# tsbertalan/openmg

Measured on AMD Instinct MI355X. Metric: V-cycles/sec, 3-D 7-point Poisson 256^3, higher is better.
Workload: dtype f64

## Files before the change

### openmg_amd/csrc/common.h

```cpp
#pragma once
#include <hip/hip_runtime.h>

#include <algorithm>
#include <array>
#include <cstdint>
#include <cstdio>
#include <cstdlib>
#include <cstring>
#include <new>
#include <stdexcept>
#include <memory>
#include <string>
#include <type_traits>
#include <utility>
#include <vector>

#include "../../include/openmg_hip.h"

#if !defined(OMG_EXPERIMENTS) && (defined(PLANE_STORE_AUX) || defined(PLANE_LA_BIG) || defined(PLANE_LA) || defined(PLANE_WAVE_SYNC) || \
                                  defined(PLANE_WSYNC_F32) || defined(S27_COEF_AUX) || defined(S27_SG) || defined(S27_WAVES) ||        \
                                  defined(MARCH_NAP_MAX) || defined(OMG_ROWBLK_NNZ) || defined(PLANE_SETPRIO))
#error "tuning switches are experiments: add -DOMG_EXPERIMENTS"
#endif

// ... 476 lines not shown
    DevBuf<int32_t> gi_ptr, gi_idx;
    DevBuf<V> gi_val;
    DevBuf<int32_t> ig_ptr, ig_idx;
    DevBuf<V> ig_val;
    DevBuf<V> y, xg;
    int sx = 0, sy = 0, sz = 0;
    DevBuf<double> sine, lambda;
    size_t bytes = 0;
    bool retain_workspace = false;
    DevBuf<double> ws_aug, ws_inv64, ws_keep;
    int64_t bs = 0;
    int K = 0;
    DevBuf<V> dinv;
    DevBuf<int32_t> lo_ptr, lo_idx, up_ptr, up_idx;
    DevBuf<V> lo_val, up_val;
    DevBuf<V> z;
    void build_chain(const HostCsr &A, const int32_t *d_ptr, const int32_t *d_idx, const double *d_val, hipStream_t s);
    void build(const HostCsr &A, hipStream_t s);
    bool build_sine(const HostCsr &A, hipStream_t s);
    void solve(const V *b, V *x, hipStream_t s) const;
    bool cube16() const;
};

constexpr int PROJECT_MAX_WG = 2048;
constexpr int PROJECT_SCRATCH = PROJECT_MAX_WG + 1;
template <typename V>
void launch_project_mean(V *x, int64_t n, double *scratch, hipStream_t s);

constexpr int MARCH_FACE_PAD = 72;
struct MarchGeom {
    int nx = 0, ny = 0, nz = 0;
    int TJ = 0, TK = 0;
    int ntj = 0, ntk = 0, n_tiles = 0;
    int T = 0, n_grp = 0;
    int n_pat = 0;
};
template <typename V>
struct MarchPlan {
    MarchGeom g;
    DevBuf<uint32_t> codes;
    DevBuf<V> coef;
    DevBuf<uint32_t> sync;
    DevBuf<int32_t> order;
    DevBuf<V> faceJ, faceK;
    bool line1 = false;
    DevBuf<V> tri;
    bool per_row = false;
    DevBuf<V> rowc;
    bool line_scan = false;
    int scan_c = 0, scan_g = 0;
    DevBuf<uint8_t> rowcode;
    DevBuf<V> face_scan;
    bool build(const omg_csr &A, hipStream_t s);
    void sweep(V *x, const V *b, hipStream_t s) const;
    bool timed_out(hipStream_t s) const;
};

struct DevCsrPlain {
    int64_t n_rows = 0, n_cols = 0, nnz = 0;
    DevBuf<int32_t> indptr, indices;
    DevBuf<double> data;
};
void galerkin_chain_device(const omg_csr &A0, int dim, const int64_t *shape, int n_restrictions, std::vector<DevCsrPlain> &A,
                           std::vector<DevCsrPlain> &R, hipStream_t s);
void galerkin_chain_semi_device(const omg_csr &A0, int dim, const int64_t *shape, int n_restrictions, const int *factors, int64_t min_size,
                                std::vector<DevCsrPlain> &A, std::vector<DevCsrPlain> &R, std::vector<int> &used, hipStream_t s);
void semicoarsen_rule(int dim, const int64_t *shape, const double *sums, const int64_t *counts, int line_axis, int level, int *factors);
void check_factors(int dim, const int64_t *ext, const int *f, int level);
HostCsr download_csr(const DevCsrPlain &M, hipStream_t s);
bool rap_aggregation_device(const DevCsrPlain &R, const DevCsrPlain &A, DevCsrPlain &C, hipStream_t s);

bool is_plain_aggregation(const omg_csr &R, int64_t nx, int64_t ny, int64_t nz, double &w);

constexpr int PLANE_EDGE = 4;
struct PlaneGeom {
    int nx = 0, ny = 0, nz = 0;
    int hx = 0;
    int z_base = 0, z_end = 0, kv0 = 0, kv1 = 0, kc_off = 0, nzc = 0;
    int TX = 0, TY = 0, LZ = 0;
    int PX = 0, PY = 0;
    int ntx = 0, nty = 0, ntz = 0, n_wg = 0;
    int threads = 0;
    size_t lds_bytes = 0;
    double c[7] = {0, 0, 0, 0, 0, 0, 0};
    double w = 0.0;
    double over = 1.0;
    bool dim2 = false;
    bool jacobi = false;
    double omega = 1.0;
    bool block = false;
    bool la2 = true;
};
template <typename V>
struct PlanePlan {
    PlaneGeom g;
    DevBuf<double> partials;
    uint32_t *status = nullptr;
    bool build(const omg_csr &A, const omg_csr &R, Ordering &ord, bool jacobi = false, double omega = 1.0);
    bool build_device(const DevCsrPlain &A, int nx, int ny, int nz, double w, Ordering &ord, bool jacobi, double omega, hipStream_t s);
    bool finish_geometry(int64_t nx, int64_t ny, int64_t nz, const double (&c)[7], double w, bool jacobi, double omega);
    void spmv(const V *x, V *y, hipStream_t s) const;
    HostCsr operator_csr() const;
    HostCsr restriction_csr() const;
    void build_slab(int nx, int ny, int nz_own, int ghost, int ghost_c, bool first, bool last, const double (&c)[7], double w);
    struct Peer {
        V *x[2] = {nullptr, nullptr};
        V *bc[2] = {nullptr, nullptr};
        int64_t shift = 0, cshift = 0;
        int planes = 0, cplanes = 0;
        int zc_lo = 0, zc_hi = 0;
        const uint32_t *wait_flag[4] = {nullptr, nullptr, nullptr, nullptr};
        uint32_t wait_seq[4] = {0, 0, 0, 0};
        bool fused_wait = true;
        uint32_t *done = nullptr;
        uint32_t *flag[2] = {nullptr, nullptr};
        uint32_t seq = 0;
        uint32_t *status = nullptr;
        uint32_t spin = 1u << 21;
    };
    struct Coarse {
        const int32_t *map = nullptr;
        V *b = nullptr;
        V *x = nullptr;
        const V *diag = nullptr;
        int first_end = 0;
        const V *e = nullptr;
    };
    void tune(V *x, V *tmp, const V *b, const Coarse &c, hipStream_t s, bool finest = true);
    float time_pair(V *x, V *tmp, const V *b, const Coarse &c, hipStream_t s, bool finest, int pairs);
    enum { PART_ALL = 0, PART_EDGE = 1, PART_INNER = 2 };
    bool can_split() const {
        return !g.dim2 && !g.block && !(g.la2 && g.threads <= 128) && (g.z_end - g.z_base) >= 3 * PLANE_EDGE;
    }
    int split_partials() const {
        const int nzo = g.z_end - g.z_base;
        return nzo >= 3 * PLANE_EDGE ? g.ntx * g.nty * (2 + (nzo - 2 * PLANE_EDGE + g.LZ - 1) / g.LZ) : g.n_wg;
    }
    struct Gate {
        const uint32_t *flag[4] = {nullptr, nullptr, nullptr, nullptr};
        uint32_t seq[4] = {0, 0, 0, 0};
        uint32_t *status = nullptr;
        uint32_t spin = 1u << 21;
    };
    bool can_gate() const { return can_split() && 2 * g.ntx * g.nty <= 192 && (g.z_end - g.z_base) >= 96; }
    int gate_lz() const;
    int gate_partials() const;
    void down(const V *x_old, V *x_new, const V *b, bool x_zero, const Coarse &c, hipStream_t s, const Peer *peer = nullptr,
              bool sweep = true, int part = PART_ALL, const Gate *gate = nullptr) const;
    void up(const V *x_old, V *x_new, const V *b, const Coarse &c, double *out, hipStream_t s, const Peer *peer = nullptr,
            bool sweep = true, int part = PART_ALL, const Gate *gate = nullptr) const;
};

template <typename V>
struct TailUp {
    const PlaneGeom *top = nullptr, *mid = nullptr;
    const V *x_old = nullptr, *b = nullptr, *mid_x_old = nullptr, *mid_b = nullptr;
    V *x_new = nullptr, *mid_x_new = nullptr;
    const int32_t *cmap = nullptr;
    const V *cb = nullptr;
    V *cx = nullptr;
    const double *tables = nullptr, *lambda = nullptr;
    bool sweep = true;
};
bool tail_up_level(const PlaneGeom &g, int nxc, int nyc, int nzc);
template <typename V>
void launch_tail_up(const TailUp<V> &u, hipStream_t s);
// ... 123 lines not shown
```

### openmg_amd/csrc/plane.hip

```cpp
#include <algorithm>
#include <array>
#include <atomic>
#include <cmath>
#include <cstring>
#include <map>
#include <mutex>
#include <thread>
#include <type_traits>

#include "common.h"
#include "peer_wait.h"
#include "sine_cube16.h"

#if defined(OMG_PLANE_STAMPS) || defined(OMG_PLANE_DBGARGS)
#define OMG_PLANE_DBG_ON 1
#endif

namespace omg {
namespace {

#ifndef PLANE_STORE_AUX
#define PLANE_STORE_AUX 2
#endif
typedef unsigned v2u __attribute__((ext_vector_type(2)));
// ... 166 lines not shown
__device__ __forceinline__ void quotients(const V (&n)[4], V c, V r, bool fast, V (&q)[4]) {
    if (sizeof(V) == 8 && fast) {
        bool bad = false;
#pragma unroll
        for (int i = 0; i < 4; ++i) {
            const V q0 = n[i] * r;
            q[i] = madd(madd(-c, q0, n[i]), r, q0);
            bad = bad || !plain_numerator(n[i]);
        }
        if (__builtin_amdgcn_ballot_w64(bad) == 0) return;
    }
#pragma unroll
    for (int i = 0; i < 4; ++i) q[i] = n[i] / c;
}

template <typename V>
struct Inline {
    V imx, ipx, imy, ipy;
};
template <typename V>
__device__ __forceinline__ Inline<V> in_line(int rule, const P2<V> &O, V nb) {
    Inline<V> r;
    r.imx = rule ? O.x : nb;
    r.ipx = rule ? O.y : O.x;
    r.imy = rule ? O.y : O.x;
    r.ipy = rule ? nb : O.y;
    return r;
}

__device__ __forceinline__ void peer_done(uint32_t *done, uint32_t n_wg, uint32_t *const (&flag)[2], uint32_t seq) {
    __builtin_amdgcn_fence(__ATOMIC_RELEASE, "workgroup");
    __syncthreads();
    if (threadIdx.x == 0) {
        const uint32_t before = __hip_atomic_fetch_add(done, 1u, __ATOMIC_RELAXED, __HIP_MEMORY_SCOPE_AGENT);
        if (before == n_wg - 1) {
            __hip_atomic_store(done, 0u, __ATOMIC_RELAXED, __HIP_MEMORY_SCOPE_AGENT);
            for (int i = 0; i < 2; ++i)
                if (flag[i]) __hip_atomic_store(flag[i], seq, __ATOMIC_RELAXED, __HIP_MEMORY_SCOPE_SYSTEM);
        }
    }
}
__global__ void plane_wait_kernel(const uint32_t *f0, const uint32_t *f1, const uint32_t *f2, const uint32_t *f3,
                                  uint32_t s0, uint32_t s1, uint32_t s2, uint32_t s3, uint32_t *status, uint32_t spin) {
    if (threadIdx.x == 0) {
        peer_wait(f0, s0, status, spin);
        peer_wait(f1, s1, status, spin);
        peer_wait(f2, s2, status, spin);
        peer_wait(f3, s3, status, spin);
    }
}

template <typename V, int MODE, bool NORM, bool XZ, int LA, bool PEER = false, int MAXT = 512, bool FIRST = false, bool SWEEP = true, bool MIRROR = false>
__global__ __launch_bounds__(MAXT) void plane_kernel(const PlaneKArgs<V> a) {
    static_assert(!MIRROR || (MODE == 1 && !PEER && !FIRST && !XZ), "mirrored march: up passes of whole grids");
#ifdef OMG_PLANE_STAMPS
    const unsigned long long st_entry = __builtin_amdgcn_s_memtime();
#endif
    extern __shared__ __attribute__((aligned(16))) unsigned char plane_smem[];
    V *const lds = reinterpret_cast<V *>(plane_smem);
    __shared__ double s_red[8];
    __shared__ int s_step[8];
    if (threadIdx.x < 8) s_step[threadIdx.x] = 0;

    const int PX = a.PX, PY = a.PY;
    const int S = 2 * PX + 4;
    const int BUF = (2 * PY + 2) * S;
    const int t = int(threadIdx.x);
    const bool live = t < PX * PY;
    const int px = live ? t % PX : 0, py = live ? t / PX : 0;
    int L = int(blockIdx.x);
    int nwg = int(gridDim.x);
    const bool edge_wg = !PEER && a.edge_wg0 > 0 && L >= a.edge_wg0;
    if (!PEER && a.edge_wg0 > 0) {
        if (edge_wg) { L -= a.edge_wg0; nwg = 1; }
        else nwg = a.edge_wg0;
    }
    if ((nwg & 7) == 0) L = (L & 7) * (nwg >> 3) + (L >> 3);
    const int nxy = a.ntx * a.nty;
    const int tz = L / nxy, rem = L - tz * nxy;
    const int ty = rem / a.ntx, tx = rem - ty * a.ntx;
    const int z0 = edge_wg ? (tz ? a.z_end - PLANE_EDGE : a.z_base) : a.zc_base + tz * a.zc_stride;
    const int z1 = edge_wg ? z0 + PLANE_EDGE : min(a.zc_end, z0 + a.zc_len);
    const int q = tx * a.TXq + px - 1;
    const int ja = ty * a.TY + 2 * py - 4;
    const bool vx0 = live && q >= 0 && 2 * q < a.hx, vx1 = live && q >= 0 && 2 * q + 1 < a.hx;
    const bool vl[2] = {ja >= 0 && ja < a.ny, ja + 1 >= 0 && ja + 1 < a.ny};
    const bool inner = live && px >= 1 && px <= PX - 2 && py >= 2 && py <= PY - 3;
    const int ps = a.ny * a.hx;
    const int lb[2] = {ja * a.hx + 2 * q, (ja + 1) * a.hx + 2 * q};

    const __amdgpu_buffer_rsrc_t xs = __builtin_amdgcn_make_buffer_rsrc(const_cast<V *>(a.x_old), 0, a.vec_bytes, 0x00020000);
    const __amdgpu_buffer_rsrc_t bs = __builtin_amdgcn_make_buffer_rsrc(const_cast<V *>(a.b), 0, a.vec_bytes, 0x00020000);
    const __amdgpu_buffer_rsrc_t ws = __builtin_amdgcn_make_buffer_rsrc(a.x_new, 0, a.vec_bytes, 0x00020000);
    const __amdgpu_buffer_rsrc_t es = __builtin_amdgcn_make_buffer_rsrc(const_cast<V *>(MODE == 1 ? a.ec : a.cdiag), 0, a.cvec_bytes, 0x00020000);
    const __amdgpu_buffer_rsrc_t ms = __builtin_amdgcn_make_buffer_rsrc(const_cast<int32_t *>(a.cmap), 0, a.cmap_bytes, 0x00020000);

    constexpr int W = int(sizeof(V));
    const bool vcell = vl[0] && vx0;
    V c1a = ja > 0 ? a.c1 : V(0);
    V c5b = ja + 2 < a.ny ? a.c5 : V(0);
    V c2x = q > 0 ? a.c2 : V(0);
    V c4x = 2 * q + 1 < a.hx ? a.c4 : V(0);
    V c4y = 2 * q + 2 < a.hx ? a.c4 : V(0);
    unsigned lbo[2] = {vcell ? unsigned(lb[0] * W) : unsigned(OOB), vcell ? unsigned(lb[1] * W) : unsigned(OOB)};
    unsigned lso[2] = {(vcell && inner) ? unsigned(lb[0] * W) : unsigned(OOB), (vcell && inner) ? unsigned(lb[1] * W) : unsigned(OOB)};
    asm volatile("" : "+v"(c1a), "+v"(c5b), "+v"(c2x), "+v"(c4x), "+v"(c4y));
    asm volatile("" : "+v"(lbo[0]), "+v"(lbo[1]), "+v"(lso[0]), "+v"(lso[1]));
    const bool oddx = (a.hx & 1) != 0;

    auto head = [&](int l, int v, int rule, V km, V jm, V im) -> V {
        V sum = madd(a.c0, km, V(0));
        sum = madd(l == 0 ? c1a : a.c1, jm, sum);
        return madd((v == 0 && rule == 0) ? c2x : a.c2, im, sum);
    };
    auto tail = [&](int l, int v, int rule, V sum, V d, V ip, V jp, V kp) -> V {
        sum = madd(a.c3, d, sum);
        sum = madd(rule == 0 ? a.c4 : (v == 0 ? c4x : c4y), ip, sum);
        sum = madd(l == 1 ? c5b : a.c5, jp, sum);
        return madd(a.c6, kp, sum);
    };

    auto zphys = [&](int k) -> int { return MIRROR ? a.nz - 1 - k : k; };
    auto cplane = [&](int kc) -> int { return MIRROR ? (a.nz / 2 - 1 + a.kc_off) - kc : kc + a.kc_off; };
    auto plane_off = [&](int colour, int k) -> unsigned {
        return (k >= a.kv0 && k < a.kv1) ? unsigned(((colour ? a.nr : 0) + zphys(k) * ps) * W) : unsigned(OOB);
    };
    auto fetch = [&](const __amdgpu_buffer_rsrc_t &rs, int colour, int k, int l) -> P2<V> {
        unsigned po = plane_off(colour, k);
        asm volatile("" : "+s"(po));
        return bload2(rs, int(lbo[l] + po), V(0));
    };
    auto fetch_at = [&](const __amdgpu_buffer_rsrc_t &rs, unsigned po, int l) -> P2<V> { return bload2(rs, int(lbo[l] + po), V(0)); };
    auto fetch_x = [&](int colour, int k, int l) -> P2<V> {
        if (XZ) return {V(0), V(0)};
        return fetch(xs, colour, k, l);
    };
    constexpr int XAUX = sizeof(V) == 8 ? PLANE_STORE_AUX : 0;
    auto put_pair = [&](const __amdgpu_buffer_rsrc_t &rs, unsigned off, const P2<V> &v) {
#ifdef OMG_PLANE_DBG_ON
        if (a.dbg & 1) return;
#endif
        if (oddx) {
            bstore1<XAUX>(rs, int(off), v.x);
            bstore1<XAUX>(rs, int(vx1 ? off + unsigned(W) : unsigned(OOB)), v.y);
        } else {
            bstore2(rs, int(off), v, true);
        }
    };
    const bool vcoarse = vcell && (MODE == 1 || inner);
    const int cbase = (ja >> 1) * a.nxc + 2 * q;
    unsigned cb4 = vcoarse ? unsigned(cbase * 4) : unsigned(OOB);
    unsigned lmx = vcoarse ? 0u : unsigned(OOB), lmy = (vcoarse && vx1) ? 0u : unsigned(OOB);
    asm volatile("" : "+v"(cb4), "+v"(lmx), "+v"(lmy));
    const v2u none = {unsigned(OOB), unsigned(OOB)};
    auto slots_request = [&](int kc, bool want) -> v2u {
        kc = cplane(kc);
        const bool ok = want && a.cmap && kc >= 0 && kc < a.nzc;
        return __builtin_amdgcn_raw_buffer_load_b64(ms, int(cb4 + (ok ? unsigned(kc * a.nyc * a.nxc * 4) : unsigned(OOB))), 0, 0);
    };
    auto slots_commit = [&](const v2u &m, int kc, bool want) -> v2u {
        kc = cplane(kc);
        const bool ok = want && kc >= 0 && kc < a.nzc;
        const unsigned u = ok ? 0u : unsigned(OOB), cn = ok ? unsigned(kc * a.nyc * a.nxc * W) : 0u;
        const unsigned s0_ = a.cmap ? m.x * unsigned(W) : cn + cb4 * unsigned(W / 4), s1_ = a.cmap ? m.y * unsigned(W) : cn + cb4 * unsigned(W / 4) + unsigned(W);
        return v2u{s0_ | lmx | u, s1_ | lmy | u};
    };
    auto coarse_slots = [&](int kc) -> v2u { return slots_commit(slots_request(kc, true), kc, true); };
    auto coarse_vals = [&](const v2u &sl) -> P2<V> { return {bload1(es, int(sl.x), V(0)), bload1(es, int(sl.y), V(0))}; };
    auto prolonged = [&](const P2<V> &x, const P2<V> &e) -> P2<V> {
        return {x.x + madd(a.wp, e.x, V(0)), x.y + madd(a.wp, e.y, V(0))};
    };

    const V rc3 = refined_rcp(a.c3);
    const bool fast = a.fast_div != 0;
    const int row_a = 1 + 2 * py, col = 2 + 2 * px;
    const int idx[2] = {row_a * S + col, (row_a + 1) * S + col};
    for (int i = t; i < 6 * BUF; i += int(blockDim.x)) lds[i] = V(0);
    if (((PEER && a.fused_wait) || edge_wg) && t == 0) {
#pragma unroll
        for (int i = 0; i < 4; ++i) peer_wait(a.wait_flag[i], a.wait_seq[i], a.status, a.spin);
    }
    __syncthreads();
    int pside = 0;
    if (PEER) {
        const bool lo = z0 < a.z_base + 2 * PEER_CPLANES, hi = z1 > a.z_end - 2 * PEER_CPLANES;
        pside = (lo && a.peer_x[0] ? 1 : 0) | (hi && a.peer_x[1] ? 2 : 0) | (lo && a.peer_bc[0] ? 4 : 0) | (hi && a.peer_bc[1] ? 8 : 0);
    }
    auto peer_store = [&](int k, int base, const P2<V> (&v)[2]) {
#pragma unroll
        for (int side = 0; side < 2; ++side) {
            const bool hit = side == 0 ? (pside & 1) && k < z0 + PEER_PLANES && k < a.z_base + PEER_PLANES
                                       : (pside & 2) && k >= z1 - PEER_PLANES && k >= a.z_end - PEER_PLANES;
            if (!hit) continue;
            V *px = a.peer_x[side];
            asm volatile("" : "+s"(px));
            const __amdgpu_buffer_rsrc_t pw = __builtin_amdgcn_make_buffer_rsrc(px ? px : a.x_new, 0, px ? a.vec_bytes : 0u, 0x00020000);
            int sh = side == 0 ? a.peer_shift : -a.peer_shift;
            asm volatile("" : "+s"(sh));
#pragma unroll
            for (int l = 0; l < 2; ++l)
                if (vl[l] && vx0) bstore2<PEER_AUX>(pw, (base + sh + lb[l]) * int(sizeof(V)), v[l], vx1);
        }
    };
    int CO_side = 0;
    const __amdgpu_buffer_rsrc_t bcs = __builtin_amdgcn_make_buffer_rsrc(a.bc, 0, a.bc ? a.cvec_bytes : 0u, 0x00020000);
    auto coarse_store = [&](const v2u &sl, const P2<V> &co, const P2<V> &cx, auto PB) {
        bstore1<0>(bcs, int(sl.x), co.x);
        bstore1<0>(bcs, int(sl.y), co.y);
        if (FIRST && a.xc) {
            const __amdgpu_buffer_rsrc_t xcs = __builtin_amdgcn_make_buffer_rsrc(a.xc, 0, a.cvec_bytes, 0x00020000);
            bstore1<0>(xcs, int(sl.x), cx.x);
            bstore1<0>(xcs, int(sl.y), cx.y);
        }
        if (PEER && decltype(PB)::value) {
#pragma unroll
            for (int side = 0; side < 2; ++side) {
                if (!(CO_side & (1 << side))) continue;
                V *pb = a.peer_bc[side];
                int sh = side == 0 ? a.peer_cshift : -a.peer_cshift;
                asm volatile("" : "+s"(pb), "+s"(sh));
                const __amdgpu_buffer_rsrc_t pwb = __builtin_amdgcn_make_buffer_rsrc(pb, 0, a.cvec_bytes, 0x00020000);
                bstore1<PEER_AUX>(pwb, sl.x < unsigned(OOB) ? int(sl.x) + sh * W : OOB, co.x);
                bstore1<PEER_AUX>(pwb, sl.y < unsigned(OOB) ? int(sl.y) + sh * W : OOB, co.y);
            }
        }
    };

    const P2<V> zero2 = {V(0), V(0)};
    P2<V> XR[3][2], XB[5][2], BR[3][2], BB[2], LXB[LA][2], LXR[LA][2], LBR[LA][2], LBB[LA][2], RB[2];
#pragma unroll
    for (int l = 0; l < 2; ++l) {
#pragma unroll
        for (int p = 0; p < 3; ++p) { XR[p][l] = zero2; BR[p][l] = zero2; }
#pragma unroll
        for (int p = 0; p < 5; ++p) XB[p][l] = zero2;
        BB[l] = zero2;
        RB[l] = zero2;
    }
    P2<V> ACC = zero2;
    P2<V> CO = zero2, CX = zero2;
    v2u SLd = none, SLo = none;
    v2u SLt = {0u, 0u};
    int SLt_kc = -1;
    P2<V> DG = zero2, DGt = zero2;
    P2<V> E0 = zero2, E1n = zero2, Et = zero2;
    v2u SLn = none;
    double sq = 0.0, sqy = 0.0;

    const int s0 = z0 - 2;
    constexpr bool RES = MODE == 0 || NORM;
    {
        P2<V> em = zero2;
        if (MODE == 1) {
            const v2u sl0 = coarse_slots(s0 >> 1), slm = coarse_slots((s0 >> 1) - 1);
            SLt_kc = (s0 >> 1) + 1;
            SLt = slots_request(SLt_kc, true);
            E0 = coarse_vals(sl0);
            em = coarse_vals(slm);
        }
#pragma unroll
        for (int l = 0; l < 2; ++l) {
            XB[0][l] = fetch_x(1, s0, l);
            XB[1][l] = RES ? fetch_x(1, s0 - 1, l) : zero2;
            if (MODE == 1) {
                XB[0][l] = prolonged(XB[0][l], E0);
                XB[1][l] = prolonged(XB[1][l], em);
            }
#pragma unroll
            for (int d = 0; d < LA; ++d) {
                LXB[d][l] = fetch_x(1, s0 + d + 1, l);
                LXR[d][l] = (RES || d > 0) ? fetch_x(0, s0 + d, l) : zero2;
                LBR[d][l] = (RES || d > 0) ? fetch(bs, 0, s0 + d, l) : zero2;
                LBB[d][l] = zero2;
            }
            if (live) lds_put(lds + (0 * 2 + (s0 & 1)) * BUF + idx[l], XB[0][l]);
        }
    }
    __syncthreads();

#ifdef OMG_PLANE_STAMPS
    unsigned long long st_mem = 0, st_cmp = 0, st_bar = 0, st_top = 0, st_B = 0, st_C = 0, st_t = __builtin_amdgcn_s_memtime();
#define PLANE_STAMP(acc) { const unsigned long long now_ = __builtin_amdgcn_s_memtime(); acc += now_ - st_t; st_t = now_; }
#else
#define PLANE_STAMP(acc)
#endif
    static_assert(!(PEER && LA == 2), "the two-step loop has no boundary steps");
#ifndef PLANE_WSYNC_F32
#define PLANE_WSYNC_F32 0
#endif
    constexpr bool WSYNC = PLANE_WAVE_SYNC && (sizeof(V) == 8 || PLANE_WSYNC_F32);
    int n_waves = int(blockDim.x) >> 6;
    asm volatile("" : "+s"(n_waves));
    const int my_wave = t >> 6, reach = (PX + 63) >> 6;
    auto publish = [&](int cnt) {
        __builtin_amdgcn_fence(__ATOMIC_RELEASE, "workgroup");
        if ((t & 63) == 0) __hip_atomic_store(&s_step[my_wave], cnt, __ATOMIC_RELAXED, __HIP_MEMORY_SCOPE_WORKGROUP);
    };
    auto await = [&](int cnt) {
        if ((t & 63) == 0) {
            for (int o = max(0, my_wave - reach); o <= min(n_waves - 1, my_wave + reach); ++o)
                for (unsigned polls = 0; __hip_atomic_load(&s_step[o], __ATOMIC_RELAXED, __HIP_MEMORY_SCOPE_WORKGROUP) < cnt; ++polls) {
                    if (polls >= WAVE_SYNC_SPIN) {
                        if (a.status) __hip_atomic_fetch_or(a.status, 2u, __ATOMIC_RELAXED, __HIP_MEMORY_SCOPE_AGENT);
                        break;
                    }
                    __builtin_amdgcn_s_sleep(1);
                }
        }
        __builtin_amdgcn_fence(__ATOMIC_ACQUIRE, "workgroup");
    };
    auto step = [&](auto PARC, const int s, auto PB) {
        constexpr bool PEER_STEP = PEER && decltype(PB)::value;
        const int par = PARC;
        const int set = LA == 2 ? par : 0;
#pragma unroll
        for (int l = 0; l < 2; ++l) {
            asm volatile("" : "+v"(LXB[set][l].x), "+v"(LXB[set][l].y), "+v"(LXR[set][l].x), "+v"(LXR[set][l].y));
            asm volatile("" : "+v"(LBR[set][l].x), "+v"(LBR[set][l].y), "+v"(LBB[set][l].x), "+v"(LBB[set][l].y));
        }
#ifdef OMG_PLANE_STAMPS
        asm volatile("s_waitcnt vmcnt(0)" ::: "memory");
        PLANE_STAMP(st_mem)
#endif
        if (MODE == 1) {
            E1n.x = par ? Et.x : E1n.x; E1n.y = par ? Et.y : E1n.y;
            const v2u sl = slots_commit(SLt, SLt_kc, true);
            SLn.x = par ? SLn.x : sl.x; SLn.y = par ? SLn.y : sl.y;
        } else {
            const v2u sl = slots_commit(SLt, SLt_kc, true);
            SLd.x = par ? SLd.x : sl.x; SLd.y = par ? SLd.y : sl.y;
            if (FIRST) { DG.x = par ? DGt.x : DG.x; DG.y = par ? DGt.y : DG.y; }
        }
#pragma unroll
        for (int l = 0; l < 2; ++l) {
            XB[4][l] = XB[3][l]; XB[3][l] = XB[2][l]; XB[2][l] = XB[1][l]; XB[1][l] = XB[0][l];
            XR[2][l] = XR[1][l]; XR[1][l] = XR[0][l];
            BR[2][l] = BR[1][l]; BR[1][l] = BR[0][l];
            if (MODE == 1) {
                XB[0][l] = prolonged(LXB[set][l], par ? E1n : E0);
                XR[0][l] = prolonged(LXR[set][l], E0);
            } else {
                XB[0][l] = LXB[set][l];
                XR[0][l] = LXR[set][l];
            }
            BR[0][l] = LBR[set][l];
            BB[l] = LBB[set][l];
        }
        if (PEER_STEP && inner && (((pside & 1) && s < z0 + PEER_PLANES + 2) || ((pside & 2) && s >= z1 - PEER_PLANES + 1))) {
            if (s - 1 >= z0 && s - 1 < z1) peer_store(s - 1, (s - 1) * ps, XR[1]);
            if (s - 2 >= z0 && s - 2 < z1) peer_store(s - 2, a.nr + (s - 2) * ps, XB[3]);
        }
        if (MODE == 1) {
            E0.x = par ? E1n.x : E0.x; E0.y = par ? E1n.y : E0.y;
            SLt_kc = (s >> 1) + 2;
            SLt = slots_request(SLt_kc, par != 0);
            Et = coarse_vals(par ? none : SLn);
        } else {
            SLt_kc = (s - 1) >> 1;
            SLt = slots_request(SLt_kc, par != 0);
            if (FIRST) DGt = coarse_vals((par || !a.cdiag) ? none : SLd);
        }
        {
            unsigned pXB = plane_off(1, s + LA + 1), pR = plane_off(0, s + LA), pBB = plane_off(1, s + LA - 1);
            {
                const bool past = s + LA > z1 + (RES ? 1 : 0);
                const int cfirst = z0 - ((RES && SWEEP) ? 1 : 0), clast = z1 - ((RES && SWEEP) ? 0 : 1);
                if (past) { pXB = unsigned(OOB); pR = unsigned(OOB); }
                if (s + LA - 1 < cfirst || s + LA - 1 > clast) pBB = unsigned(OOB);
            }
            asm volatile("" : "+s"(pXB), "+s"(pR), "+s"(pBB));
#ifdef OMG_PLANE_DBG_ON
            if (a.dbg & 16) {
                if (s + LA + 1 < z0 || s + LA + 1 >= z1) pXB = unsigned(OOB);
                if (s + LA < z0 || s + LA >= z1) pR = unsigned(OOB);
                if (s + LA - 1 < z0 || s + LA - 1 >= z1) pBB = unsigned(OOB);
            }
            if (a.dbg & 4) { pXB = unsigned(OOB); }
            unsigned pR_b = pR;
            if (a.dbg & 4) pR = unsigned(OOB);
            if (a.dbg & 8) { pR_b = unsigned(OOB); pBB = unsigned(OOB); }
#else
            const unsigned pR_b = pR;
#endif
#pragma unroll
            for (int l = 0; l < 2; ++l) {
                LXB[set][l] = XZ ? zero2 : fetch_at(xs, pXB, l);
                LXR[set][l] = XZ ? zero2 : fetch_at(xs, pR, l);
                LBR[set][l] = fetch_at(bs, pR_b, l);
                LBB[set][l] = fetch_at(bs, pBB, l);
            }
        }
        if (MODE == 0 && !par && s - 3 >= z0 && s - 3 < z1) {
#ifdef OMG_PLANE_DBG_ON
            if (!(a.dbg & 2))
#endif
            coarse_store(SLo, CO, CX, PB);
        }

        PLANE_STAMP(st_top)
        if (WSYNC) await(s - s0);
        PLANE_STAMP(st_bar)
#ifdef PLANE_SETPRIO
        __builtin_amdgcn_s_setprio(PLANE_SETPRIO);
#endif
        P2<V> d_jm = zero2, d_jp = zero2;
        V d_nb[2] = {V(0), V(0)};
        P2<V> rb[2] = {zero2, zero2};
        if (live) {
            const V *const E1 = lds + (0 * 2 + par) * BUF;
            const V *const E2 = lds + (1 * 2 + par) * BUF;
            const V *const E3 = lds + (2 * 2 + par) * BUF;
            const bool pvB = s >= a.kv0 && s < a.kv1, pvC = s - 1 >= a.kv0 && s - 1 < a.kv1;
            const bool liveT = s > z0 && s <= z1;
            const bool liveB = RES || (s >= z0 - 1 && s <= z1);
            const bool liveC = SWEEP ? (RES ? s >= z0 : liveT) : liveT;
            if (SWEEP && liveB) {
                const P2<V> jm = lds_pair(E1 + idx[0] - S), jp = lds_pair(E1 + idx[1] + S);
                const P2<V> o0 = XB[1][0], o1 = XB[1][1];
                V num[4], quo[4];
#pragma unroll
                for (int l = 0; l < 2; ++l) {
                    const int rule = (l + par + (MIRROR ? 1 : 0)) & 1;
                    const P2<V> O = l ? o1 : o0, Ojm = l ? o0 : jm, Ojp = l ? jp : o1;
                    const Inline<V> n = in_line(rule, O, E1[idx[l] + (rule ? 2 : -1)]);
                    const P2<V> D = XR[0][l], Bv = BR[0][l], Km = XB[MIRROR ? 0 : 2][l], Kp = XB[MIRROR ? 2 : 0][l];
                    num[2 * l] = Bv.x - tail(l, 0, rule, head(l, 0, rule, Km.x, Ojm.x, n.imx), D.x, n.ipx, Ojp.x, Kp.x);
                    num[2 * l + 1] = Bv.y - tail(l, 1, rule, head(l, 1, rule, Km.y, Ojm.y, n.imy), D.y, n.ipy, Ojp.y, Kp.y);
                }
                quotients(num, a.c3, rc3, fast, quo);
#pragma unroll
                for (int l = 0; l < 2; ++l) {
                    XR[0][l].x = XR[0][l].x + quo[2 * l];
                    XR[0][l].y = XR[0][l].y + quo[2 * l + 1];
                }
                if (!pvB) {
                    asm volatile("" ::: "memory");
                    XR[0][0] = zero2; XR[0][1] = zero2;
                }
            }
            if ((SWEEP || MODE == 1) && s - 1 >= z0 && s - 1 < z1) {
                const unsigned base = unsigned(zphys(s - 1) * ps * W);
#pragma unroll
                for (int l = 0; l < 2; ++l) put_pair(ws, lso[l] + base, XR[1][l]);
            }
            PLANE_STAMP(st_B)
            if (liveC) {
                const P2<V> jm = lds_pair(E2 + idx[0] - S), jp = lds_pair(E2 + idx[1] + S);
                const P2<V> o0 = XR[1][0], o1 = XR[1][1];
                V num[4], quo[4], hd[4];
                Inline<V> nl[2];
                P2<V> Jp[2];
#pragma unroll
                for (int l = 0; l < 2; ++l) {
                    const int rule = (l + par + (MIRROR ? 1 : 0)) & 1;
                    const P2<V> O = l ? o1 : o0, Ojm = l ? o0 : jm, Ojp = l ? jp : o1;
                    nl[l] = in_line(rule, O, E2[idx[l] + (rule ? 2 : -1)]);
                    Jp[l] = Ojp;
                    const P2<V> D = XB[2][l], Bv = BB[l], Km = XR[MIRROR ? 0 : 2][l], Kp = XR[MIRROR ? 2 : 0][l];
                    hd[2 * l] = head(l, 0, rule, Km.x, Ojm.x, nl[l].imx);
                    hd[2 * l + 1] = head(l, 1, rule, Km.y, Ojm.y, nl[l].imy);
                    num[2 * l] = Bv.x - tail(l, 0, rule, hd[2 * l], D.x, nl[l].ipx, Ojp.x, Kp.x);
                    num[2 * l + 1] = Bv.y - tail(l, 1, rule, hd[2 * l + 1], D.y, nl[l].ipy, Ojp.y, Kp.y);
                }
                if (SWEEP) quotients(num, a.c3, rc3, fast, quo);
#pragma unroll
                for (int l = 0; l < 2; ++l) {
                    if (!SWEEP) {
                        rb[l].x = num[2 * l];
                        rb[l].y = num[2 * l + 1];
                        continue;
                    }
                    XB[2][l].x = XB[2][l].x + quo[2 * l];
                    XB[2][l].y = XB[2][l].y + quo[2 * l + 1];
// ... 679 lines not shown
    if (SWEEP && JAC) {
        constexpr int wx = BX + 2, wy = BY + 2, np = wx * wy, NI = (np + NT - 1) / NT;
        for (int i = t; i < vol; i += NT) XN[i] = V(0);
        __syncthreads();
#pragma unroll
        for (int n = 0; n < NI; ++n) {
            const int p = t + n * NT;
            const int li = 2 + p % wx, lj = 2 + p / wx;
            const int gi = i0 + li, gj = j0 + lj;
            if (p >= np || !in_grid(gi, gj)) continue;
            const int l = lj * EX + li;
            XN[l] = X[l] + a.omega * block_quotient(B[l] - row(l), a.c3, rc3, fast);
        }
        __syncthreads();
        Y = XN;
    } else if (SWEEP) {
        sweep(0, std::integral_constant<int, 2>());
        __syncthreads();
        sweep(1, std::integral_constant<int, 1>());
        __syncthreads();
    }
    constexpr int NB = (BX * BY + NT - 1) / NT;
    double sq = 0.0;
#pragma unroll
    for (int n = 0; n < NB; ++n) {
        const int c = t + n * NT;
        const int li = 3 + c % BX, lj = 3 + c / BX;
        const int gi = i0 + li, gj = j0 + lj;
        if (c >= BX * BY || gi >= a.nx || gj >= a.ny) continue;
        const int l = lj * EX + li;
        if (SWEEP || MODE == 1) a.x_new[slot_of(gi, gj)] = Y[l];
        if (MODE == 0 || NORM) {
            const V res = B[l] - row_of(Y, l);
            if (MODE == 0) E[c] = res;
            if (NORM) sq = fma(double(res), double(res), sq);
        }
    }
    if (MODE == 0) {
        __syncthreads();
        constexpr int hx = BX / 2, hy = BY / 2, NCC = (hx * hy + NT - 1) / NT;
#pragma unroll
        for (int n = 0; n < NCC; ++n) {
            const int c = t + n * NT;
            const int I = c % hx, J = c / hx;
            const int GI = (bi * BX >> 1) + I, GJ = (bj * BY >> 1) + J;
            if (c >= hx * hy || GI >= a.nxc || GJ >= a.nyc) continue;
            V acc = V(0);
#pragma unroll
            for (int d = 0; d < 4; ++d) acc = madd(a.w, E[(2 * J + (d >> 1)) * BX + 2 * I + (d & 1)], acc);
            const int ce = GJ * a.nxc + GI;
            a.bc[a.cmap ? a.cmap[ce] : ce] = acc;
        }
    }
    if (NORM) {
#pragma unroll
        for (int off = 32; off > 0; off >>= 1) sq += __shfl_down(sq, off, 64);
        if ((t & 63) == 0) s_red[t >> 6] = sq;
        __syncthreads();
        if (t == 0) {
            double tot = 0.0;
            for (int wv = 0; wv < NT / 64; ++wv) tot += s_red[wv];
            a.partials[blockIdx.x] = tot;
        }
    }
}

int env_int3(const char *name, int out[3]) {
    const char *e = getenv(name);
    if (!e || !e[0]) return 0;
    return sscanf(e, "%d,%d,%d", &out[0], &out[1], &out[2]) == 3 ? 1 : 0;
}

inline int round_up(int v, int m) { return (v + m - 1) / m * m; }

inline void small_level_switches(PlaneGeom &g) {
    auto env = [](const char *name, long long dflt) { const char *e = getenv(name); return e && e[0] ? atoll(e) : dflt; };
    const bool whole = g.z_base == 0 && g.z_end == g.nz && g.kv0 == 0 && g.kv1 == g.nz;
    g.block = env("OMG_PLANE_BLOCK", 1) != 0 && whole && int64_t(g.nx) * g.ny * g.nz <= env("OMG_PLANE_BLOCK_CELLS", int64_t(64) * 64 * 64);
    g.la2 = env("OMG_PLANE_LA2", 1) != 0;
}

void choose_tiles(PlaneGeom &g, size_t value_bytes, int model = 0, std::vector<std::array<int, 3>> *more = nullptr, int keep = 0) {
    const int nzo = g.z_end - g.z_base;
    auto set = [&](int TX, int TY, int LZ) {
        g.TX = TX; g.TY = TY; g.LZ = LZ;
        g.PX = TX / 4 + 2; g.PY = TY / 2 + 4;
        g.ntx = (g.nx + TX - 1) / TX; g.nty = (g.ny + TY - 1) / TY; g.ntz = (nzo + LZ - 1) / LZ;
        g.n_wg = g.ntx * g.nty * g.ntz;
        g.threads = round_up(g.PX * g.PY, 64);
        g.lds_bytes = size_t(6) * size_t(2 * g.PY + 2) * size_t(2 * g.PX + 4) * value_bytes;
    };
    int forced[3];
    if (env_int3("OMG_PLANE_TILE", forced)) {
        const int TX = std::max(4, round_up(forced[0], 4)), TY = std::max(2, round_up(forced[1], 2)), LZ = std::max(2, round_up(forced[2], 2));
        set(TX, TY, LZ);
        if (g.threads <= 512 && g.lds_bytes <= size_t(160) * 1024) return;
    }
    std::vector<std::pair<double, std::array<int, 3>>> all;
    for (int ntx = 1; ntx <= (g.nx + 3) / 4; ++ntx) {
        const int TX = round_up((g.nx + ntx - 1) / ntx, 4);
        if ((g.nx + TX - 1) / TX != ntx) continue;
        for (int nty = 1; nty <= g.ny / 2; ++nty) {
            const int TY = round_up((g.ny + nty - 1) / nty, 2);
            if ((g.ny + TY - 1) / TY != nty) continue;
            const int thr = round_up((TX / 4 + 2) * (TY / 2 + 4), 64);
            if (thr > 512) continue;
            if (size_t(6) * size_t(TY + 10) * size_t(TX / 2 + 8) * value_bytes > size_t(150) * 1024) continue;
            for (int ntz = 1; ntz <= nzo / 2; ++ntz) {
                const int LZ = round_up((nzo + ntz - 1) / ntz, 2);
                if ((nzo + LZ - 1) / LZ != ntz) continue;
                double cost;
                if (model == 0) {
                    const double rounds = std::ceil(double(ntx) * nty * ntz / 256.0);
                    cost = rounds * (LZ + 4) * (thr + 192.0);
                } else {
                    const int waves = thr / 64;
                    const size_t lds = size_t(6) * size_t(TY + 10) * size_t(TX / 2 + 8) * value_bytes;
                    const int per_cu = std::max(1, std::min(8 / waves, int(size_t(160) * 1024 / lds)));
                    const int simd = (waves * per_cu + 3) / 4;
                    const double rounds = std::ceil(double(ntx) * nty * ntz / (256.0 * per_cu));
                    cost = rounds * (LZ + 4) * (256.0 * simd + 192.0);
                }
                all.push_back({cost, {TX, TY, LZ}});
            }
        }
    }
    if (all.empty()) { g.TX = 0; return; }
    std::stable_sort(all.begin(), all.end(), [](const auto &u, const auto &v) { return u.first < v.first; });
    set(all[0].second[0], all[0].second[1], all[0].second[2]);
    if (more)
        for (size_t i = 1; i < all.size() && int(more->size()) < keep; ++i) more->push_back(all[i].second);
}

constexpr int TILE2_SHAPES[3][2] = {{64, 32}, {32, 16}, {16, 8}};
void choose_tile2d(PlaneGeom &g, size_t value_bytes) {
    int pick = 2;
    for (int i = 0; i < 3; ++i) {
        const int64_t n = int64_t((g.nx + TILE2_SHAPES[i][0] - 1) / TILE2_SHAPES[i][0]) * ((g.ny + TILE2_SHAPES[i][1] - 1) / TILE2_SHAPES[i][1]);
        if (n >= 128) { pick = i; break; }
    }
    g.block = false;
    g.TX = TILE2_SHAPES[pick][0]; g.TY = TILE2_SHAPES[pick][1]; g.LZ = 1;
    g.ntx = (g.nx + g.TX - 1) / g.TX; g.nty = (g.ny + g.TY - 1) / g.TY; g.ntz = 1;
    g.n_wg = g.ntx * g.nty;
    g.threads = 256;
    const size_t vol = size_t(g.TX + 6) * size_t(g.TY + 6);
    g.lds_bytes = ((g.jacobi ? 3 : 2) * vol + std::max(size_t(g.TX) * g.TY, size_t(g.TX / 2 + 4) * size_t(g.TY / 2 + 4))) * value_bytes;
    (void)pick;
}

}

template <typename V>
bool PlanePlan<V>::build(const omg_csr &A, const omg_csr &R, Ordering &ord, bool jacobi, double omega) {
    {
        const char *e = getenv("OMG_PLANE");
        if (e && e[0] == '0') return false;
    }
    const int64_t n = A.n_rows;
    if (n < 8 || n != A.n_cols || uint64_t(n) * sizeof(V) >= (uint64_t(1) << 31)) return false;
    auto has = [&](int64_t r, int64_t c) {
        for (int64_t p = A.indptr[r]; p < A.indptr[r + 1]; ++p)
            if (A.indices[p] == c) return true;
        return false;
    };
    int64_t nx = n;
    for (int64_t r = 1; r < n; ++r)
        if (!has(r, r - 1)) { nx = r; break; }
    if (nx < 2 || n % nx) return false;
    const int64_t lines = n / nx;
    int64_t ny = lines;
    for (int64_t q = 1; q < lines; ++q)
        if (!has(q * nx, (q - 1) * nx)) { ny = q; break; }
    if (lines % ny) return false;
    const int64_t nz = lines / ny;
    const bool dim2 = nz == 1;
    if ((nx & 1) || (ny & 1) || (!dim2 && (nz & 1)) || ny < 2) return false;
    if (jacobi && !dim2) return false;
    {
        const char *e = experiment_env("OMG_PLANE_2D");
        if (dim2 && e && e[0] == '0') return false;
    }
    const int64_t sj = nx, sk = nx * ny;
    bool havec[7] = {false, false, false, false, false, false, false};
    double c[7] = {0, 0, 0, 0, 0, 0, 0};
    auto slot_of = [&](int64_t r, int64_t col) -> int {
        const int64_t i = r % nx, jl = (r / nx) % ny, kl = r / sk, off = col - r;
        if (off == 0) return 3;
        if (off == -1 && i > 0) return 2;
        if (off == 1 && i + 1 < nx) return 4;
        if (off == -sj && jl > 0) return 1;
        if (off == sj && jl + 1 < ny) return 5;
        if (off == -sk && kl > 0) return 0;
        if (off == sk && kl + 1 < nz) return 6;
        return -1;
    };
    {
        const int64_t probe = std::min<int64_t>(n - 1, sk + sj + 1);
        for (int64_t r : {probe, int64_t(0), n - 1}) {
            for (int64_t p = A.indptr[r]; p < A.indptr[r + 1]; ++p) {
// ... 165 lines not shown
            if (off == 0) sl = 3;
            else if (off == -1 && i > 0) sl = 2;
            else if (off == 1 && i + 1 < nx) sl = 4;
            else if (off == -sj && jl > 0) sl = 1;
            else if (off == sj && jl + 1 < ny) sl = 5;
            else if (off == -sk && kl > 0) sl = 0;
            else if (off == sk && kl + 1 < nz) sl = 6;
            if (sl < 0) return false;
            if (!havec[sl]) { havec[sl] = true; c[sl] = val[q]; }
        }
    }
    if (dim2) havec[0] = havec[6] = true;
    for (int e = 0; e < 7; ++e)
        if (!havec[e]) return false;
    if (!(std::fabs(c[3]) > 0.0) || !std::isfinite(c[3])) return false;
    DevBuf<unsigned long long> d_err(1);
    OMG_HIP(hipMemsetAsync(d_err.p, 0xFF, sizeof(unsigned long long), s));
    hipLaunchKernelGGL(plane_check_kernel, dim3(unsigned((n + 255) / 256)), dim3(256), 0, s, A.indptr.p, A.indices.p, A.data.p, nx, ny, nz,
                       c[0], c[1], c[2], c[3], c[4], c[5], c[6], d_err.p);
    OMG_HIP(hipGetLastError());
    unsigned long long err = 0;
    OMG_HIP(hipMemcpyAsync(&err, d_err.p, sizeof(err), hipMemcpyDeviceToHost, s));
    OMG_HIP(hipStreamSynchronize(s));
    if (err != ~0ull) return false;
    ord = Ordering();
    if (jacobi) {
        ord.identity = true;
        ord.sets = {0, n};
    } else {
        ord.identity = false;
        ord.sets = {0, n / 2, n};
        ord.closed_form = 2; ord.cf_nx = nx; ord.cf_ny = ny; ord.cf_nz = nz;
    }
    return finish_geometry(nx, ny, nz, c, w, jacobi, omega);
}

template <typename V>
void PlanePlan<V>::build_slab(int nx, int ny, int nz_own, int ghost, int ghost_c, bool first, bool last, const double (&c)[7], double w) {
    OMG_REQUIRE(nx >= 2 && ny >= 2 && nz_own >= 2 && !(nx & 1) && !(ny & 1) && !(nz_own & 1) && !(ghost & 1) && ghost >= 4 && ghost_c >= 2,
                "plane slab: extents must be even, at least four ghost planes (two on the coarse slab)");
    g = PlaneGeom();
    g.nx = nx; g.ny = ny; g.nz = nz_own + 2 * ghost; g.hx = nx / 2;
    for (int e = 0; e < 7; ++e) g.c[e] = double(V(c[e]));
    g.w = double(V(w));
    g.z_base = ghost; g.z_end = ghost + nz_own;
    g.kv0 = first ? ghost : 0;
    g.kv1 = last ? ghost + nz_own : g.nz;
    g.nzc = nz_own / 2 + 2 * ghost_c;
    g.kc_off = ghost_c - ghost / 2;
    OMG_REQUIRE(uint64_t(nx) * ny * g.nz * sizeof(V) < (uint64_t(1) << 31), "plane slab: vector exceeds 2 GiB");
    choose_tiles(g, sizeof(V));
    small_level_switches(g);
    OMG_REQUIRE(g.TX > 0 && g.threads <= 512, "plane slab: no tiling");
    partials.alloc(size_t(std::max(g.n_wg, split_partials())) + SUM_FOLD);
}

template <typename V>
void PlanePlan<V>::tune(V *x, V *tmp, const V *b, const Coarse &c, hipStream_t s, bool finest) {
    {
        const char *e = experiment_env("OMG_PLANE_TUNE");
        int forced[3];
        if ((e && e[0] == '0') || env_int3("OMG_PLANE_TILE", forced)) return;
    }
    if (g.dim2 || int64_t(g.nx) * g.ny * (g.z_end - g.z_base) < (int64_t(1) << 21)) return;
    static const int keep = [] { const char *e = experiment_env("OMG_PLANE_TUNE_K"); return e ? std::max(0, atoi(e)) : 0; }();
    static const bool debug = [] { const char *e = experiment_env("OMG_PLANE_TUNE_DEBUG"); return e && e[0] == '1'; }();
    std::vector<PlaneGeom> cand;
    {
        std::vector<std::array<int, 3>> more0, more1;
        PlaneGeom g0 = g, g1 = g;
        choose_tiles(g0, sizeof(V), 0, &more0, keep);
        choose_tiles(g1, sizeof(V), 1, &more1, keep);
        auto add = [&](const PlaneGeom &q) {
            if (q.TX <= 0 || q.threads > 512) return;
            for (const PlaneGeom &c : cand)
                if (c.TX == q.TX && c.TY == q.TY && c.LZ == q.LZ) return;
            cand.push_back(q);
        };
        add(g);
        add(g0);
        add(g1);
        auto from = [&](const std::array<int, 3> &t) {
            PlaneGeom q = g;
            q.TX = t[0]; q.TY = t[1]; q.LZ = t[2];
            q.PX = q.TX / 4 + 2; q.PY = q.TY / 2 + 4;
            const int nzo = q.z_end - q.z_base;
            q.ntx = (q.nx + q.TX - 1) / q.TX; q.nty = (q.ny + q.TY - 1) / q.TY; q.ntz = (nzo + q.LZ - 1) / q.LZ;
            q.n_wg = q.ntx * q.nty * q.ntz;
            q.threads = round_up(q.PX * q.PY, 64);
            q.lds_bytes = size_t(6) * size_t(2 * q.PY + 2) * size_t(2 * q.PX + 4) * sizeof(V);
            return q;
        };
        for (const auto &t : more0) add(from(t));
        for (const auto &t : more1) add(from(t));
        if (const char *e = experiment_env("OMG_PLANE_TUNE_EXTRA")) {
            const char *q = e;
            while (*q) {
                int t3[3];
                if (sscanf(q, "%d,%d,%d", &t3[0], &t3[1], &t3[2]) == 3 && t3[0] >= 4 && t3[1] >= 2 && t3[2] >= 2) {
                    PlaneGeom c = from({round_up(t3[0], 4), round_up(t3[1], 2), round_up(t3[2], 2)});
                    if (c.lds_bytes <= size_t(160) * 1024) add(c);
                }
                while (*q && *q != ';') ++q;
                if (*q == ';') ++q;
            }
        }
    }
    if (cand.size() < 2) return;
    static std::mutex mu;
    static std::map<std::array<int, 8>, std::array<int, 3>> decided;
    const std::array<int, 8> key = {g.nx, g.ny, g.nz, g.z_base, g.z_end, int(sizeof(V)), finest ? 1 : 0, g.kv1 - g.kv0};
    auto adopt = [&](const std::array<int, 3> &t) {
        for (const PlaneGeom &c : cand)
            if (c.TX == t[0] && c.TY == t[1] && c.LZ == t[2]) { g = c; break; }
        partials.alloc(size_t(std::max(g.n_wg, split_partials())) + SUM_FOLD);
    };
    {
        std::lock_guard<std::mutex> lock(mu);
        const auto it = decided.find(key);
        if (it != decided.end()) {
            adopt(it->second);
            return;
        }
    }
    int max_wg = 0;
    for (const PlaneGeom &c : cand) max_wg = std::max(max_wg, c.n_wg);
    partials.alloc(size_t(std::max(max_wg, split_partials())) + SUM_FOLD);
    hipEvent_t e0, e1;
    OMG_HIP(hipEventCreate(&e0));
    OMG_HIP(hipEventCreate(&e1));
    float best = 0.0f;
    size_t pick = 0;
    for (size_t i = 0; i < cand.size(); ++i) {
        g = cand[i];
        down(x, tmp, b, !finest, c, s);
        up(tmp, x, b, c, finest ? partials.p : nullptr, s);
        OMG_HIP(hipEventRecord(e0, s));
        for (int r = 0; r < 2; ++r) {
            down(x, tmp, b, !finest, c, s);
            up(tmp, x, b, c, finest ? partials.p : nullptr, s);
        }
        OMG_HIP(hipEventRecord(e1, s));
        OMG_HIP(hipEventSynchronize(e1));
        float ms = 0.0f;
        OMG_HIP(hipEventElapsedTime(&ms, e0, e1));
        if (debug)
            fprintf(stderr, "[plane tune] %dx%dx%d%s: tile %3d x %3d x %3d  %4d workgroups of %3d threads  %7.1f us per down + up\n", g.nx, g.ny, g.nz,
                    finest ? " (finest)" : "", g.TX, g.TY, g.LZ, g.n_wg, g.threads, 1e3 * ms / 2);
        if (i == 0 || ms < best) { best = ms; pick = i; }
    }
    (void)hipEventDestroy(e0);
    (void)hipEventDestroy(e1);
    std::array<int, 3> chosen = {cand[pick].TX, cand[pick].TY, cand[pick].LZ};
    {
        std::lock_guard<std::mutex> lock(mu);
        chosen = decided.emplace(key, chosen).first->second;
    }
    adopt(chosen);
}

template <typename V>
float PlanePlan<V>::time_pair(V *x, V *tmp, const V *b, const Coarse &c, hipStream_t s, bool finest, int pairs) {
    hipEvent_t e0, e1;
    OMG_HIP(hipEventCreate(&e0));
    OMG_HIP(hipEventCreate(&e1));
    down(x, tmp, b, !finest, c, s);
    up(tmp, x, b, c, finest ? partials.p : nullptr, s);
    OMG_HIP(hipEventRecord(e0, s));
    for (int r = 0; r < pairs; ++r) {
        down(x, tmp, b, !finest, c, s);
        up(tmp, x, b, c, finest ? partials.p : nullptr, s);
    }
    OMG_HIP(hipEventRecord(e1, s));
// ... 478 lines not shown
```

Before: 3955.

## Shrink plane tile y-halo to one row-pair and load edge rows via ring lanes

The plane smoother tile shrinks its y halo from two row-pairs per side to one, so PY drops from TY/2+4 to TY/2+2 threads and both the LDS footprint and the thread count fall. The edge threads (py==0 and py==PY-1) now fetch the single extra neighbouring row from global memory each plane, and prolong it in MODE 1. They pipeline it the same way as the other rows and write it into a new LDS ring slot. This cuts redundant halo compute and frees resources for occupancy or larger tiles, at the cost of extra per-plane loads and coarse-map lookups on edge lanes. Tile geometry math is consolidated into PlaneGeom helpers.

After: 3924. About the same (-0.8%).

```diff
diff --git a/openmg_amd/csrc/common.h b/openmg_amd/csrc/common.h
--- a/openmg_amd/csrc/common.h
+++ b/openmg_amd/csrc/common.h
@@ -582,6 +582,21 @@
     int ntx = 0, nty = 0, ntz = 0, n_wg = 0;
     int threads = 0;
     size_t lds_bytes = 0;
+    static int tile_px(int TX) { return TX / 4 + 2; }
+    static int tile_py(int TY) { return TY / 2 + 2; }
+    static int tile_threads(int TX, int TY) { return (tile_px(TX) * tile_py(TY) + 63) / 64 * 64; }
+    static size_t tile_lds(int TX, int TY, size_t value_bytes) {
+        return size_t(6) * size_t(2 * tile_py(TY) + 2) * size_t(2 * tile_px(TX) + 4) * value_bytes;
+    }
+    void set_tile(int TX_, int TY_, int LZ_, size_t value_bytes) {
+        TX = TX_; TY = TY_; LZ = LZ_;
+        PX = tile_px(TX); PY = tile_py(TY);
+        const int nzo = z_end - z_base;
+        ntx = (nx + TX - 1) / TX; nty = (ny + TY - 1) / TY; ntz = (nzo + LZ - 1) / LZ;
+        n_wg = ntx * nty * ntz;
+        threads = tile_threads(TX, TY);
+        lds_bytes = tile_lds(TX, TY, value_bytes);
+    }
     double c[7] = {0, 0, 0, 0, 0, 0, 0};
     double w = 0.0;
     double over = 1.0;
diff --git a/openmg_amd/csrc/plane.hip b/openmg_amd/csrc/plane.hip
--- a/openmg_amd/csrc/plane.hip
+++ b/openmg_amd/csrc/plane.hip
@@ -272,10 +272,10 @@
     const int z0 = edge_wg ? (tz ? a.z_end - PLANE_EDGE : a.z_base) : a.zc_base + tz * a.zc_stride;
     const int z1 = edge_wg ? z0 + PLANE_EDGE : min(a.zc_end, z0 + a.zc_len);
     const int q = tx * a.TXq + px - 1;
-    const int ja = ty * a.TY + 2 * py - 4;
+    const int ja = ty * a.TY + 2 * py - 2;
     const bool vx0 = live && q >= 0 && 2 * q < a.hx, vx1 = live && q >= 0 && 2 * q + 1 < a.hx;
     const bool vl[2] = {ja >= 0 && ja < a.ny, ja + 1 >= 0 && ja + 1 < a.ny};
-    const bool inner = live && px >= 1 && px <= PX - 2 && py >= 2 && py <= PY - 3;
+    const bool inner = live && px >= 1 && px <= PX - 2 && py >= 1 && py <= PY - 2;
     const int ps = a.ny * a.hx;
     const int lb[2] = {ja * a.hx + 2 * q, (ja + 1) * a.hx + 2 * q};
 
@@ -297,6 +297,12 @@
     asm volatile("" : "+v"(c1a), "+v"(c5b), "+v"(c2x), "+v"(c4x), "+v"(c4y));
     asm volatile("" : "+v"(lbo[0]), "+v"(lbo[1]), "+v"(lso[0]), "+v"(lso[1]));
     const bool oddx = (a.hx & 1) != 0;
+    constexpr bool RING = (MODE == 0 || NORM) && !XZ;
+    const int je = py == 0 ? ja - 1 : ja + 2;
+    const bool vring = RING && live && (py == 0 || py == PY - 1) && je >= 0 && je < a.ny && vx0;
+    unsigned lbe = vring ? unsigned((je * a.hx + 2 * q) * W) : unsigned(OOB);
+    int idxe = vring ? (py == 0 ? 0 : 2 * PY + 1) * (2 * PX + 4) + 2 + 2 * px : -1;
+    if (RING) asm volatile("" : "+v"(lbe), "+v"(idxe));
 
     auto head = [&](int l, int v, int rule, V km, V jm, V im) -> V {
         V sum = madd(a.c0, km, V(0));
@@ -342,19 +348,27 @@
     unsigned cb4 = vcoarse ? unsigned(cbase * 4) : unsigned(OOB);
     unsigned lmx = vcoarse ? 0u : unsigned(OOB), lmy = (vcoarse && vx1) ? 0u : unsigned(OOB);
     asm volatile("" : "+v"(cb4), "+v"(lmx), "+v"(lmy));
+    constexpr bool RING_E = RING && MODE == 1;
+    unsigned cb4e = vring ? unsigned((cbase + (py == 0 ? -a.nxc : a.nxc)) * 4) : unsigned(OOB);
+    unsigned lme = vring ? 0u : unsigned(OOB);
+    if (RING_E) asm volatile("" : "+v"(cb4e), "+v"(lme));
     const v2u none = {unsigned(OOB), unsigned(OOB)};
-    auto slots_request = [&](int kc, bool want) -> v2u {
+    auto slots_request_at = [&](unsigned cb, int kc, bool want) -> v2u {
         kc = cplane(kc);
         const bool ok = want && a.cmap && kc >= 0 && kc < a.nzc;
-        return __builtin_amdgcn_raw_buffer_load_b64(ms, int(cb4 + (ok ? unsigned(kc * a.nyc * a.nxc * 4) : unsigned(OOB))), 0, 0);
-    };
-    auto slots_commit = [&](const v2u &m, int kc, bool want) -> v2u {
+        return __builtin_amdgcn_raw_buffer_load_b64(ms, int(cb + (ok ? unsigned(kc * a.nyc * a.nxc * 4) : unsigned(OOB))), 0, 0);
+    };
+    auto slots_commit_at = [&](unsigned cb, unsigned mx, unsigned my, const v2u &m, int kc, bool want) -> v2u {
         kc = cplane(kc);
         const bool ok = want && kc >= 0 && kc < a.nzc;
         const unsigned u = ok ? 0u : unsigned(OOB), cn = ok ? unsigned(kc * a.nyc * a.nxc * W) : 0u;
-        const unsigned s0_ = a.cmap ? m.x * unsigned(W) : cn + cb4 * unsigned(W / 4), s1_ = a.cmap ? m.y * unsigned(W) : cn + cb4 * unsigned(W / 4) + unsigned(W);
-        return v2u{s0_ | lmx | u, s1_ | lmy | u};
-    };
+        const unsigned s0_ = a.cmap ? m.x * unsigned(W) : cn + cb * unsigned(W / 4), s1_ = a.cmap ? m.y * unsigned(W) : cn + cb * unsigned(W / 4) + unsigned(W);
+        return v2u{s0_ | mx | u, s1_ | my | u};
+    };
+    auto slots_request = [&](int kc, bool want) -> v2u { return slots_request_at(cb4, kc, want); };
+    auto slots_commit = [&](const v2u &m, int kc, bool want) -> v2u { return slots_commit_at(cb4, lmx, lmy, m, kc, want); };
+    auto ring_slots_request = [&](int kc, bool want) -> v2u { return slots_request_at(cb4e, kc, want); };
+    auto ring_slots_commit = [&](const v2u &m, int kc, bool want) -> v2u { return slots_commit_at(cb4e, lme, lme | lmy, m, kc, want); };
     auto coarse_slots = [&](int kc) -> v2u { return slots_commit(slots_request(kc, true), kc, true); };
     auto coarse_vals = [&](const v2u &sl) -> P2<V> { return {bload1(es, int(sl.x), V(0)), bload1(es, int(sl.y), V(0))}; };
     auto prolonged = [&](const P2<V> &x, const P2<V> &e) -> P2<V> {
@@ -435,6 +449,10 @@
     P2<V> DG = zero2, DGt = zero2;
     P2<V> E0 = zero2, E1n = zero2, Et = zero2;
     v2u SLn = none;
+    P2<V> LXE[LA], EE = zero2;
+    v2u SLE = {0u, 0u};
+#pragma unroll
+    for (int d = 0; d < LA; ++d) LXE[d] = zero2;
     double sq = 0.0, sqy = 0.0;
 
     const int s0 = z0 - 2;
@@ -447,6 +465,23 @@
             SLt = slots_request(SLt_kc, true);
             E0 = coarse_vals(sl0);
             em = coarse_vals(slm);
+            if (RING_E) {
+                EE = coarse_vals(ring_slots_commit(ring_slots_request(s0 >> 1, true), s0 >> 1, true));
+                SLE = ring_slots_request(SLt_kc, true);
+            }
+        }
+        if (RING) {
+            unsigned po = plane_off(1, s0);
+            asm volatile("" : "+s"(po));
+            P2<V> xe = bload2(xs, int(lbe + po), V(0));
+            if (MODE == 1) xe = prolonged(xe, EE);
+            if (idxe >= 0) lds_put(lds + (0 * 2 + (s0 & 1)) * BUF + idxe, xe);
+#pragma unroll
+            for (int d = 0; d < LA; ++d) {
+                unsigned pd = plane_off(1, s0 + d + 1);
+                asm volatile("" : "+s"(pd));
+                LXE[d] = bload2(xs, int(lbe + pd), V(0));
+            }
         }
 #pragma unroll
         for (int l = 0; l < 2; ++l) {
@@ -508,6 +543,7 @@
             asm volatile("" : "+v"(LXB[set][l].x), "+v"(LXB[set][l].y), "+v"(LXR[set][l].x), "+v"(LXR[set][l].y));
             asm volatile("" : "+v"(LBR[set][l].x), "+v"(LBR[set][l].y), "+v"(LBB[set][l].x), "+v"(LBB[set][l].y));
         }
+        if (RING) asm volatile("" : "+v"(LXE[set].x), "+v"(LXE[set].y));
 #ifdef OMG_PLANE_STAMPS
         asm volatile("s_waitcnt vmcnt(0)" ::: "memory");
         PLANE_STAMP(st_mem)
@@ -536,6 +572,14 @@
             BR[0][l] = LBR[set][l];
             BB[l] = LBB[set][l];
         }
+        if (RING) {
+            static_assert(!RING_E || !FIRST, "the ring line's coarse values: the step's parity is a constant");
+            if (idxe >= 0) lds_put(lds + (0 * 2 + (par ^ 1)) * BUF + idxe, MODE == 1 ? prolonged(LXE[set], EE) : LXE[set]);
+            if (RING_E) {
+                if (!par) EE = coarse_vals(ring_slots_commit(SLE, SLt_kc, true));
+                else SLE = ring_slots_request((s >> 1) + 2, true);
+            }
+        }
         if (PEER_STEP && inner && (((pside & 1) && s < z0 + PEER_PLANES + 2) || ((pside & 2) && s >= z1 - PEER_PLANES + 1))) {
             if (s - 1 >= z0 && s - 1 < z1) peer_store(s - 1, (s - 1) * ps, XR[1]);
             if (s - 2 >= z0 && s - 2 < z1) peer_store(s - 2, a.nr + (s - 2) * ps, XB[3]);
@@ -579,6 +623,7 @@
                 LBR[set][l] = fetch_at(bs, pR_b, l);
                 LBB[set][l] = fetch_at(bs, pBB, l);
             }
+            if (RING) LXE[set] = bload2(xs, int(lbe + pXB), V(0));
         }
         if (MODE == 0 && !par && s - 3 >= z0 && s - 3 < z1) {
 #ifdef OMG_PLANE_DBG_ON
@@ -1424,14 +1469,7 @@
 
 void choose_tiles(PlaneGeom &g, size_t value_bytes, int model = 0, std::vector<std::array<int, 3>> *more = nullptr, int keep = 0) {
     const int nzo = g.z_end - g.z_base;
-    auto set = [&](int TX, int TY, int LZ) {
-        g.TX = TX; g.TY = TY; g.LZ = LZ;
-        g.PX = TX / 4 + 2; g.PY = TY / 2 + 4;
-        g.ntx = (g.nx + TX - 1) / TX; g.nty = (g.ny + TY - 1) / TY; g.ntz = (nzo + LZ - 1) / LZ;
-        g.n_wg = g.ntx * g.nty * g.ntz;
-        g.threads = round_up(g.PX * g.PY, 64);
-        g.lds_bytes = size_t(6) * size_t(2 * g.PY + 2) * size_t(2 * g.PX + 4) * value_bytes;
-    };
+    auto set = [&](int TX, int TY, int LZ) { g.set_tile(TX, TY, LZ, value_bytes); };
     int forced[3];
     if (env_int3("OMG_PLANE_TILE", forced)) {
         const int TX = std::max(4, round_up(forced[0], 4)), TY = std::max(2, round_up(forced[1], 2)), LZ = std::max(2, round_up(forced[2], 2));
@@ -1445,9 +1483,10 @@
         for (int nty = 1; nty <= g.ny / 2; ++nty) {
             const int TY = round_up((g.ny + nty - 1) / nty, 2);
             if ((g.ny + TY - 1) / TY != nty) continue;
-            const int thr = round_up((TX / 4 + 2) * (TY / 2 + 4), 64);
+            const int thr = PlaneGeom::tile_threads(TX, TY);
             if (thr > 512) continue;
-            if (size_t(6) * size_t(TY + 10) * size_t(TX / 2 + 8) * value_bytes > size_t(150) * 1024) continue;
+            const size_t lds = PlaneGeom::tile_lds(TX, TY, value_bytes);
+            if (lds > size_t(150) * 1024) continue;
             for (int ntz = 1; ntz <= nzo / 2; ++ntz) {
                 const int LZ = round_up((nzo + ntz - 1) / ntz, 2);
                 if ((nzo + LZ - 1) / LZ != ntz) continue;
@@ -1457,7 +1496,6 @@
                     cost = rounds * (LZ + 4) * (thr + 192.0);
                 } else {
                     const int waves = thr / 64;
-                    const size_t lds = size_t(6) * size_t(TY + 10) * size_t(TX / 2 + 8) * value_bytes;
                     const int per_cu = std::max(1, std::min(8 / waves, int(size_t(160) * 1024 / lds)));
                     const int simd = (waves * per_cu + 3) / 4;
                     const double rounds = std::ceil(double(ntx) * nty * ntz / (256.0 * per_cu));
@@ -1789,13 +1827,7 @@
         add(g1);
         auto from = [&](const std::array<int, 3> &t) {
             PlaneGeom q = g;
-            q.TX = t[0]; q.TY = t[1]; q.LZ = t[2];
-            q.PX = q.TX / 4 + 2; q.PY = q.TY / 2 + 4;
-            const int nzo = q.z_end - q.z_base;
-            q.ntx = (q.nx + q.TX - 1) / q.TX; q.nty = (q.ny + q.TY - 1) / q.TY; q.ntz = (nzo + q.LZ - 1) / q.LZ;
-            q.n_wg = q.ntx * q.nty * q.ntz;
-            q.threads = round_up(q.PX * q.PY, 64);
-            q.lds_bytes = size_t(6) * size_t(2 * q.PY + 2) * size_t(2 * q.PX + 4) * sizeof(V);
+            q.set_tile(t[0], t[1], t[2], sizeof(V));
             return q;
         };
         for (const auto &t : more0) add(from(t));
```
